# jamesmshihua/DiffusionPolicyOptimization

Measured on AMD Instinct MI355X. Metric: env-steps/sec + PPO-updates/sec, hopper-v2 64 envs 20 DDPM steps, 1/2/4/8 GPU, higher is better.
Workload: dtype bf16; 1 GPU; hopper-medium-v2 DPPO fine-tune iteration: 64 envs/GPU x 500 chunks (Ta=4), K=20 DDPM steps (K'=10), 5 PPO epochs x minibatch 50000, bf16 denoiser, synthetic linear env; env=synthetic, global_envs=64, chunks_per_rollout=500, parallelism=single GPU, batch_semantics=global minibatch 50000 rows = the reference's (50000 per rank)

## Files before the change

### diffusionpolicyoptimization_amd/_lib.py

```python
import ctypes
import os

import torch

_HERE = os.path.dirname(os.path.abspath(__file__))
LIB_PATH = os.environ.get("DPPO_LIB") or os.path.join(_HERE, "lib", "libdppo_hip.so")

DPPO_F32, DPPO_BF16, DPPO_F16 = 0, 1, 2
DPPO_ADAMW_KERAS, DPPO_ADAMW_TORCH = 0, 1
DPPO_STEP_DEFER_SAMPLER_TABLES = 0x100
DPPO_STEP_L2_FROM_PL2 = 0x200
DPPO_PPO_L2_DEFERRED = 1
DPPO_PPO_LEARN_ETA = 2
DPPO_STEP_FUSED_PACK = 0x400
DPPO_STEP_CLEAR_GRADS = 0x800
DPPO_PPO_PRECLEARED = 4
DPPO_NET_ACTOR, DPPO_NET_CRITIC = 1, 2
SCHED_COLS = 8
PRECISION = {"fp32": DPPO_F32, "f32": DPPO_F32, "bf16": DPPO_BF16, "fp16": DPPO_F16, "f16": DPPO_F16}
ACTIVATION = {"ReLU": 0, "Mish": 1}


class DppoDims(ctypes.Structure):
    _fields_ = [("obs_dim", ctypes.c_int32), ("action_dim", ctypes.c_int32), ("horizon_steps", ctypes.c_int32),
# ... 38 lines not shown
    "dppo_rollout_enqueue_tagged": (_I, [_DIMS, _I, _P, _P, _P, _P, _P, _I, _U64, _U64, _I, _I, _F, _F, _F, _P, _P,
                                         _P, ctypes.c_uint32, _P, _P]),
    "dppo_sampler_stream_bytes": (_I, [_DIMS, _I, ctypes.POINTER(ctypes.c_int64), ctypes.POINTER(ctypes.c_int)]),
    "dppo_sampler_layout": (_I, [_DIMS, _I, _I, ctypes.POINTER(ctypes.c_int)]),
    "dppo_sampler_max_in_flight": (_I, [_DIMS, _I, _I, ctypes.POINTER(ctypes.c_int)]),
    "dppo_sampler_plan": (_I, [_DIMS, _I, _I, ctypes.POINTER(ctypes.c_int)]),
    "dppo_sampler_release_stream": (_I, [_P]),
    "dppo_kernel_timing": (_I, [_I]),
    "dppo_kernel_timing_name": (ctypes.c_char_p, [_I]),
    "dppo_kernel_timing_read": (_I, [_I, _P, _P]),
    "dppo_logprob": (_I, [_DIMS, _I, _P, _P, _P, _P, _I, _F, _I, _P, _P, _P]),
    "dppo_critic_forward": (_I, [_DIMS, _I, _P, _P, _I, _P, _P]),
    "dppo_reward_scale_workspace_doubles": (_SZ, [_I, _I]),
    "dppo_reward_scale": (_I, [_P, _P, _P, _P, _P, _I, _I, _D, _D, _D, _P]),
    "dppo_reward_scale_moments": (_I, [_P, _P, _P, _P, _P, _I, _I, _D, _P]),
    "dppo_reward_scale_apply": (_I, [_P, _P, _I, _I, _D, _D, _P]),
    "dppo_reward_scale_per_env": (_I, [_P, _P, _P, _P, _I, _P, _P, _I, _I, _D, _D, _D, _P, _P]),
    "dppo_reward_scale_per_env_moments": (_I, [_P, _P, _P, _P, _P, _I, _I, _D, _P]),
    "dppo_reward_scale_per_env_apply": (_I, [_P, _P, _I, _I, _I, _D, _D, _P, _P]),
    "dppo_gae": (_I, [_P, _P, _P, _P, _I, _I, _D, _D, _D, _P, _P, _P]),
    "dppo_ppo_workspace_bytes": (_SZ, [_DIMS, _I, _I]),
    "dppo_ppo_plan": (_I, [_DIMS, _I, _I, _I, ctypes.POINTER(ctypes.c_int)]),
    "dppo_ppo_plan_act": (_I, [_DIMS, _I, _I, _I, _I, ctypes.POINTER(ctypes.c_int)]),
    "dppo_ppo_adv_stats": (_I, [_P, _I64, _I, _U64, _I, _I64, _I, _P, _P, _P]),
    "dppo_ppo_adv_stats_all": (_I, [_P, _I64, _I, _U64, _I, _I, _I64, _I, _P, _P]),
    "dppo_ppo_minibatch": (_I, [_DIMS, _I, ctypes.POINTER(DppoPpoHparams), _P, _P, _P, _P, _P, _P, _P, _P, _P,
                               _I64, _U64, _I, _I64, _I, _P, _P, _P, _P, _P, _P]),
    "dppo_pretrain_minibatch": (_I, [_DIMS, _I, _P, _P, _P, _P, _P, _P, _P, _P, _I, _I64, _F, _P, _P, _P, _P]),
    "dppo_ppo_minibatch_part": (_I, [_DIMS, _I, ctypes.POINTER(DppoPpoHparams), _P, _P, _P, _P, _P, _P, _P, _P,
                                    _P, _I64, _U64, _I, _I64, _I, _P, _P, _P, _P, _P, _I, _P]),
    "dppo_feistel_permute": (_I, [_I64, _I64, _I64, _U64, _I, _P, _P]),
    "dppo_adamw": (_I, [_P, _P, _P, _P, _I64, _I64, _F, _F, _F, _F, _F, _I, _P]),
    "dppo_copy_from_host": (_I, [_I, _P, _P, _P, _P]),
    "dppo_eta_step": (_I, [_P, _P, _I64, _F, _F, _F, _F, _F, _I, _F, _F, _P, _P, _I, _P, _P]),
    "dppo_pack_all": (_I, [_DIMS, _I, _P, _P, _P, _P, _P]),
    "dppo_optimizer_step": (_I, [_DIMS, _I, _P, _P, _P, _P, _I64, _I64, _F, _F, _F, _F, _F, _I, _P, _P, _P, _P, _P,
                                 _P, _I, _U64, _P]),
    "dppo_optimizer_step_ex": (_I, [_DIMS, _I, _P, _P, _P, _P, _I64, _I64, _F, _F, _F, _F, _F, _I, _P, _P, _P, _P,
                                    _P, _P, _I, _U64, _P, _P, _I, _P]),
    "dppo_grad_clip_workspace_bytes": (_SZ, [_DIMS, _I]),
    "dppo_grad_clip_scales": (_I, [_DIMS, _I, _P, _F, _P, _P, _P, _P]),
    "dppo_optimizer_step_clip": (_I, [_DIMS, _I, _P, _P, _P, _P, _I64, _I64, _F, _F, _F, _F, _F, _I, _P, _P, _P, _P,
                                      _P, _P, _I, _U64, _P, _P, _I, _P, _P, _I]),
    "dppo_ipc_region_bytes": (_SZ, [_I64]),
    "dppo_ipc_alloc": (_I, [_SZ, ctypes.POINTER(ctypes.c_void_p), _P]),
    "dppo_ipc_open": (_I, [_P, ctypes.POINTER(ctypes.c_void_p)]),
# ... 62 lines not shown
```

### diffusionpolicyoptimization_amd/csrc/dppo_update.h

```cpp
#pragma once
#include "dppo_ppo.h"

enum { EXTRA_NONE = 0, EXTRA_ONES = 1, EXTRA_ONEHOT = 2 };
struct DWItem {
    const void* XT; int Kx;
    const void* DT; int N;
    float* G;
    int extra;
    float* Gx;
    int nb;
};
enum class DWTile { ACTOR, CRITIC };
int launch_dw(DWTile tile, int precision, const DWItem* items, int n_items, const PpoWorkspace& ws, float out_scale,
              const int* rows_dev, int min_chunk_rows, hipStream_t s);
struct DWPlan { int tiles, nchunks, mchunk; };
DWPlan dw_plan(DWTile tile, const DWItem* items, int n_items, size_t ldm, int min_chunk_rows);

int launch_time_bwd(const Dims& D, int precision, const PpoWorkspace& ws, const void* packed_actor,
                    const float* actor_params, float* ga, int nb, int TS, hipStream_t s, bool l2_back = true);
int time_bwd_check(const Dims& D, int nb);
int launch_critic_l2_back(const Dims& D, int precision, const PpoWorkspace& ws, const void* packed_critic, float* gc,
                          uint32_t* zcnt, hipStream_t s);

struct ZeroArgs { void* p[4]; size_t n[4]; };
int launch_zero(const ZeroArgs& z, unsigned blocks, hipStream_t s);
enum { SCRATCH_TICKET = 0, SCRATCH_CRIT_COUNT = 1 };
int stream_scratch(hipStream_t s, int kind, size_t bytes, void** out);
```

### diffusionpolicyoptimization_amd/csrc/dw.hip

```cpp
#include "dppo_update.h"

#define DW_MAXP 8
#define DW_TN 128
constexpr int DW_LINE = 128;
#define DW_CPL (DW_LINE / 16)
#define DW_FPI (64 / DW_CPL)
#define DW_BOPB (DW_TN * DW_LINE)

template <int WK, int RC = 8> struct DWGeom {
    static constexpr int W = WK / 32;
    static constexpr int AOPB = WK * DW_LINE;
    static constexpr int SLOT = AOPB + DW_BOPB + 1024;
    static constexpr int RING0 = 160 * 1024 / SLOT < 8 ? 160 * 1024 / SLOT : 8;
    static constexpr int RING = RING0 < RC ? RING0 : RC;
    static constexpr int AI = WK / DW_FPI / W;
    static constexpr int BI = DW_TN / DW_FPI / W;
    static_assert(RING * SLOT <= 160 * 1024, "dW ring exceeds the CU's LDS");
};

struct DWProb {
    const void* XT; const void* DT; float* G; float* Gx;
    int Kx, N, extra, ktiles, ntiles;
    int nb;
};
struct DWArgs {
    DWProb p[DW_MAXP];
    int tile_start[DW_MAXP + 1];
    int nprob, nchunks, mchunk;
    float out_scale;
    size_t ldm;
    const int8_t* seg;
    const int* rows_dev;
};

typedef __attribute__((address_space(3))) void lds_void_t;

template <class P>
__device__ inline u32x4 extra_frag(int extra, int q, const int8_t* seg_lds) {
    using AT = typename P::AT;
    AT e[P::EPL];
    if (extra == EXTRA_ONES) {
#pragma unroll
        for (int i = 0; i < P::EPL; ++i) e[i] = P::cvt(1.f);
    } else {
        const uint64_t w = P::EPL == 8 ? *reinterpret_cast<const uint64_t*>(seg_lds)
                                       : (uint64_t)*reinterpret_cast<const uint32_t*>(seg_lds);
#pragma unroll
        for (int i = 0; i < P::EPL; ++i) e[i] = P::cvt((int)(int8_t)(w >> (8 * i)) == q ? 1.f : 0.f);
    }
    return __builtin_bit_cast(u32x4, e);
}

__device__ inline int dw_swz(int f, int c) { return c ^ (f & 7); }
__device__ inline u32x4 dw_lds_frag(const uint8_t* img, int f, int c) {
    return *reinterpret_cast<const u32x4*>(img + f * DW_LINE + (dw_swz(f, c) << 4));
}

template <int N>
__device__ inline void vm_wait() {
    static_assert(N >= 0 && N < 64, "vmcnt is 6 bits");
    __builtin_amdgcn_s_waitcnt((N & 15) | ((N >> 4) << 14) | (7 << 4) | (15 << 8));
}

template <class P, int WK, int RC, bool EXTRA, bool SEGLD>
__device__ __forceinline__ void dw_loop(uint8_t* smem, const DWArgs& a, const DWProb& pr, int nst, size_t m_begin,
                                        int wave, int lane, const typename P::AT* const (&srcA)[DWGeom<WK, RC>::AI],
                                        const typename P::AT* const (&srcB)[DWGeom<WK, RC>::BI],
                                        f32x4 (&acc)[4][4], f32x4 (&acce)[4]) {
    using G = DWGeom<WK, RC>;
    constexpr int BK = DW_LINE / (int)sizeof(typename P::AT);
    constexpr int OPS = G::AI + G::BI + (SEGLD ? 1 : 0);
    const int wr = wave >> 1, wc = wave & 1;
    const int fr = lane & 15, cq = lane >> 4;
    auto issue = [&](int st) {
        uint8_t* base = smem + (st % G::RING) * G::SLOT;
        const size_t off = (size_t)st * BK;
#pragma unroll
        for (int i = 0; i < G::AI; ++i)
            __builtin_amdgcn_global_load_lds((void*)(srcA[i] + off), (lds_void_t*)(base + (wave + G::W * i) * 1024), 16,
                                             0, 0);
#pragma unroll
        for (int i = 0; i < G::BI; ++i)
            __builtin_amdgcn_global_load_lds((void*)(srcB[i] + off),
                                             (lds_void_t*)(base + G::AOPB + (wave + G::W * i) * 1024), 16, 0, 0);
        if constexpr (SEGLD) {
            const int8_t* sg = a.seg + m_begin + off + 4 * (lane < BK / 4 ? lane : 0);
            __builtin_amdgcn_global_load_lds((void*)sg, (lds_void_t*)(base + G::AOPB + DW_BOPB), 4, 0, 0);
        }
    };
#pragma unroll
    for (int p = 0; p < G::RING - 1; ++p)
        if (p < nst) issue(p);
    for (int st = 0; st < nst; ++st) {
        const int ahead = nst - 1 - st;
        if (ahead >= G::RING - 2) vm_wait<(G::RING - 2) * OPS>();
        else if (ahead == 1) vm_wait<OPS>();
        else vm_wait<0>();
        __builtin_amdgcn_s_barrier();
        asm volatile("" ::: "memory");
        if (st + G::RING - 1 < nst) issue(st + G::RING - 1);
        const uint8_t* imA = smem + (st % G::RING) * G::SLOT;
        const uint8_t* imB = imA + G::AOPB;
        const int8_t* seg_lds = (const int8_t*)(imB + DW_BOPB);
#pragma unroll
        for (int ks = 0; ks < DW_LINE / 64; ++ks) {
            u32x4 A[4], B[4];
#pragma unroll
            for (int i = 0; i < 4; ++i) {
                A[i] = dw_lds_frag(imA, wr * 64 + i * 16 + fr, ks * 4 + cq);
                B[i] = dw_lds_frag(imB, wc * 64 + i * 16 + fr, ks * 4 + cq);
            }
#pragma unroll
            for (int i = 0; i < 4; ++i)
#pragma unroll
                for (int j = 0; j < 4; ++j) acc[i][j] = P::mma(A[i], B[j], acc[i][j]);
            if constexpr (EXTRA) {
                const u32x4 AE = extra_frag<P>(pr.extra, 16 * wr + fr, seg_lds + ks * P::KG + cq * P::EPL);
#pragma unroll
                for (int j = 0; j < 4; ++j) acce[j] = P::mma(AE, B[j], acce[j]);
            }
        }
    }
}

static int dw_device_cus() {
    static int n = [] {
        int dev = 0, c = 0;
        if (hipGetDevice(&dev) != hipSuccess || hipDeviceGetAttribute(&c, hipDeviceAttributeMultiprocessorCount, dev) != hipSuccess)
            c = 256;
        return c > 0 ? c : 256;
    }();
    return n;
}

template <class P, int WK, int RC>
__global__ __launch_bounds__(WK / 32 * 64) void dw_kernel(DWArgs a) {
    using AT = typename P::AT;
    using G = DWGeom<WK, RC>;
    constexpr int BK = DW_LINE / (int)sizeof(AT);
    constexpr int EPC = 16 / (int)sizeof(AT);
    __shared__ __attribute__((aligned(1024))) uint8_t smem[G::RING * G::SLOT];
    const int tid = threadIdx.x, lane = tid & 63, wave = tid >> 6;
    const int tiles_all = a.tile_start[a.nprob];
    const int total = tiles_all * a.nchunks;
    const int per = (total + 7) >> 3;
    const int lg = (int)(blockIdx.x & 7) * per + (int)(blockIdx.x >> 3);
    if (lg >= total) return;
    const int chunk = lg / tiles_all;
    const int tile = lg % tiles_all;
    int pi = 0;
    while (pi + 1 < a.nprob && tile >= a.tile_start[pi + 1]) ++pi;
    const DWProb& pr = a.p[pi];
    const int lt = tile - a.tile_start[pi];
    const int kt = lt / pr.ntiles, nt = lt % pr.ntiles;
    const int k_base = kt * WK, n_base = nt * DW_TN;
    const int wr = wave >> 1, wc = wave & 1;
    size_t lim = a.ldm, mchunk = (size_t)a.mchunk;
    if (a.rows_dev) {
        const size_t d64 = (size_t)(__builtin_amdgcn_readfirstlane(*a.rows_dev) + 63) / 64 * 64;
        lim = d64 < lim ? d64 : lim;
        mchunk = (lim + (size_t)a.nchunks * 64 - 1) / ((size_t)a.nchunks * 64) * 64;
    }
    const size_t m_begin = (size_t)chunk * mchunk;
    const size_t m_end = m_begin + mchunk < lim ? m_begin + mchunk : lim;
    if (m_begin >= m_end) return;
    const int nst = (int)((m_end - m_begin) / BK);
    const AT* XT = (const AT*)pr.XT;
    const AT* DT = (const AT*)pr.DT;
    const bool wg_extra = pr.extra != EXTRA_NONE && kt == 0;
    const int xrows = pr.extra == EXTRA_ONEHOT ? pr.nb : 1;
    const bool do_extra = wg_extra && 16 * wr < xrows;
    const bool seg_ld = wg_extra && wr == 0 && pr.extra == EXTRA_ONEHOT;

    const AT* srcA[G::AI];
    const AT* srcB[G::BI];
#pragma unroll
    for (int i = 0; i < G::AI; ++i) {
        const int f = (wave + G::W * i) * DW_FPI + lane / DW_CPL;
        const int c = dw_swz(f, lane % DW_CPL);
        int fa = k_base + f; fa = fa < pr.Kx ? fa : pr.Kx - 1;
        srcA[i] = XT + (size_t)fa * a.ldm + m_begin + c * EPC;
    }
#pragma unroll
    for (int i = 0; i < G::BI; ++i) {
        const int f = (wave + G::W * i) * DW_FPI + lane / DW_CPL;
        const int c = dw_swz(f, lane % DW_CPL);
        int fb = n_base + f; fb = fb < pr.N ? fb : pr.N - 1;
        srcB[i] = DT + (size_t)fb * a.ldm + m_begin + c * EPC;
    }
    f32x4 acc[4][4], acce[4];
#pragma unroll
    for (int i = 0; i < 4; ++i) {
        zero_acc(acce[i]);
#pragma unroll
        for (int j = 0; j < 4; ++j) zero_acc(acc[i][j]);
    }
    if (seg_ld) dw_loop<P, WK, RC, true, true>(smem, a, pr, nst, m_begin, wave, lane, srcA, srcB, acc, acce);
    else if (do_extra) dw_loop<P, WK, RC, true, false>(smem, a, pr, nst, m_begin, wave, lane, srcA, srcB, acc, acce);
    else dw_loop<P, WK, RC, false, false>(smem, a, pr, nst, m_begin, wave, lane, srcA, srcB, acc, acce);
#pragma unroll
    for (int i = 0; i < 4; ++i)
#pragma unroll
        for (int j = 0; j < 4; ++j) {
            const int n = n_base + wc * 64 + j * 16 + ccol(lane);
#pragma unroll
            for (int r = 0; r < 4; ++r) {
                const int k = k_base + wr * 64 + i * 16 + crow(lane, r);
                if (k < pr.Kx && n < pr.N) atomicAdd(pr.G + (size_t)k * pr.N + n, acc[i][j][r] * a.out_scale);
            }
        }
    if (do_extra) {
#pragma unroll
        for (int j = 0; j < 4; ++j) {
            const int n = n_base + wc * 64 + j * 16 + ccol(lane);
            if (n >= pr.N) continue;
#pragma unroll
            for (int r = 0; r < 4; ++r) {
                const int q = 16 * wr + crow(lane, r);
                if (pr.extra == EXTRA_ONES) {
                    if (q == 0) atomicAdd(pr.Gx + n, acce[j][r] * a.out_scale);
                } else if (q < pr.nb) {
                    atomicAdd(pr.Gx + (size_t)q * pr.N + n, acce[j][r] * a.out_scale);
                }
            }
        }
    }
}
template <class P>
static int launch_dw_p(const DWArgs& a, DWTile tile, hipStream_t s) {
    const int tiles = a.tile_start[a.nprob];
    const int64_t blocks = 8 * (((int64_t)tiles * a.nchunks + 7) / 8);
    if (tile == DWTile::ACTOR)
        hipLaunchKernelGGL((dw_kernel<P, 256, 8>), dim3((unsigned)blocks), dim3(DWGeom<256>::W * 64), 0, s, a);
    else
        hipLaunchKernelGGL((dw_kernel<P, 128, 3>), dim3((unsigned)blocks), dim3(DWGeom<128, 3>::W * 64), 0, s, a);
    DPPO_HIP(hipGetLastError());
    return DPPO_OK;
}

static int dw_item_tiles(DWTile tile, const DWItem& it) {
    return dppo_cdiv(it.Kx, tile == DWTile::ACTOR ? 256 : 128) * dppo_cdiv(it.N, DW_TN);
}

DWPlan dw_plan(DWTile tile, const DWItem* items, int n_items, size_t ldm, int min_chunk_rows) {
    DWPlan p = {};
    for (int i = 0; i < n_items; ++i) p.tiles += dw_item_tiles(tile, items[i]);
    const int span = (int)ldm;
    int nch = dw_device_cus() / p.tiles;
    if (nch > span / min_chunk_rows) nch = span / min_chunk_rows;
    if (nch < 1) nch = 1;
    p.mchunk = dppo_cdiv(span, nch * 64) * 64;
    p.nchunks = dppo_cdiv(span, p.mchunk);
    return p;
}

int launch_dw(DWTile tile, int precision, const DWItem* items, int n_items, const PpoWorkspace& ws, float out_scale,
              const int* rows_dev, int min_chunk_rows, hipStream_t s) {
    DPPO_CHECK(n_items >= 1 && n_items <= DW_MAXP, "dW: %d problems in one launch", n_items);
    const int tk = tile == DWTile::ACTOR ? 256 : 128;
    for (int i = 0; i < n_items; ++i)
        DPPO_CHECK(items[i].extra != EXTRA_ONEHOT || (items[i].nb >= 1 && items[i].nb <= tk / 4),
                   "dW: %d one-hot buckets on a %d-row tile", items[i].nb, tk);
    DWArgs w = {};
    for (int i = 0; i < n_items; ++i) {
        const DWItem& it = items[i];
        DWProb& p = w.p[i];
        p.XT = it.XT; p.DT = it.DT; p.G = it.G; p.Gx = it.Gx; p.Kx = it.Kx; p.N = it.N; p.extra = it.extra; p.nb = it.nb;
        p.ktiles = dppo_cdiv(it.Kx, tk); p.ntiles = dppo_cdiv(it.N, DW_TN);
        w.tile_start[i + 1] = w.tile_start[i] + dw_item_tiles(tile, it);
    }
    w.nprob = n_items;
    w.rows_dev = rows_dev;
    w.ldm = ws.ldm;
    w.seg = ws.seg;
    w.out_scale = out_scale;
    const DWPlan plan = dw_plan(tile, items, n_items, ws.ldm, min_chunk_rows);
    w.mchunk = plan.mchunk;
    w.nchunks = plan.nchunks;
    return precision == DPPO_BF16 ? launch_dw_p<PolicyBF16>(w, tile, s)
         : precision == DPPO_F16  ? launch_dw_p<PolicyF16>(w, tile, s) : launch_dw_p<PolicyF32>(w, tile, s);
}
```

### diffusionpolicyoptimization_amd/csrc/update.hip

```cpp
#include <stdlib.h>
#include <mutex>
#include <vector>
#include "dppo_update.h"

__global__ __launch_bounds__(256) void adv_stats_kernel(const float* __restrict__ adv, FeistelKey fk, int KF, int64_t start,
                                                        int rows, const int64_t* __restrict__ row_index,
                                                        double* __restrict__ stats) {
    __shared__ double sh[3][4];
    double c = 0.0, s = 0.0, s2 = 0.0;
    for (int64_t i = (int64_t)blockIdx.x * 256 + threadIdx.x; i < rows; i += (int64_t)gridDim.x * 256) {
        const uint64_t idx = minibatch_row(row_index, (uint64_t)(start + i), fk);
        if (idx >= fk.n) continue;
        const double v = adv[idx / KF];
        c += 1.0; s += v; s2 += v * v;
    }
    c = wave_sumd(c); s = wave_sumd(s); s2 = wave_sumd(s2);
    const int w = threadIdx.x >> 6;
    if ((threadIdx.x & 63) == 0) { sh[0][w] = c; sh[1][w] = s; sh[2][w] = s2; }
    __syncthreads();
    if (threadIdx.x == 0) {
        atomicAdd(stats + 0, sh[0][0] + sh[0][1] + sh[0][2] + sh[0][3]);
        atomicAdd(stats + 1, sh[1][0] + sh[1][1] + sh[1][2] + sh[1][3]);
        atomicAdd(stats + 2, sh[2][0] + sh[2][1] + sh[2][2] + sh[2][3]);
    }
// ... 273 lines not shown
extern "C" int dppo_ppo_plan(const dppo_dims* d, int precision, int rows, int mode, int* out) {
    return dppo_ppo_plan_act(d, precision, DPPO_ACT_RELU, rows, mode, out);
}

extern "C" int dppo_ppo_plan_act(const dppo_dims* d, int precision, int activation, int rows, int mode, int* out) {
    Dims D;
    int rc = dppo_check_dims(d, &D);
    if (rc) return rc;
    DPPO_CHECK(dppo_prec_ok(precision), "bad precision %d", precision);
    DPPO_CHECK(dppo_act_ok(activation), "dppo_ppo_plan_act: bad activation %d", activation);
    DPPO_CHECK(out && rows > 0, "dppo_ppo_plan: bad arguments");
    DPPO_CHECK(mode == DPPO_PLAN_TRAIN || mode == DPPO_PLAN_PRETRAIN || mode == DPPO_PLAN_LOGPROB,
               "dppo_ppo_plan: mode must be 0 (train), 1 (pretrain) or 2 (logprob)");
    const PpoWorkspace ws = make_ppo_workspace(D, precision, rows, nullptr);
    const ActorTilePlan t = actor_tile_plan(precision, D.H, D.XD, mode == DPPO_PLAN_LOGPROB ? (int64_t)rows : (int64_t)ws.ldm,
                                            activation);
    out[0] = 16 * t.mt;
    out[1] = t.waves;
    out[2] = out[3] = out[4] = out[5] = 0;
    if (mode == DPPO_PLAN_LOGPROB) return DPPO_OK;
    DWItem it[4];
    actor_dw_items(D, ws, nullptr, mode == DPPO_PLAN_PRETRAIN, false, it);
    const DWPlan pa = dw_plan(DWTile::ACTOR, it, 4, ws.ldm, mode == DPPO_PLAN_PRETRAIN ? PRETRAIN_MIN_CHUNK_ROWS : PPO_MIN_CHUNK_ROWS);
    out[2] = pa.nchunks;
    out[3] = pa.mchunk;
    if (mode == DPPO_PLAN_PRETRAIN) return DPPO_OK;
    critic_dw_items(D, ws, nullptr, it);
    const DWPlan pc = dw_plan(DWTile::CRITIC, it, 4, ws.ldm, PPO_MIN_CHUNK_ROWS);
    out[4] = pc.nchunks;
    out[5] = pc.mchunk;
    return DPPO_OK;
}

struct MinibatchArgs {
    const dppo_dims* d;
    int precision;
    const dppo_ppo_hparams* hp;
    const void* packed_ft; const void* packed_critic;
    const float *actor_params, *sched, *obs, *chains, *lp_old_mean, *advantages, *returns;
    int64_t total;
    uint64_t perm_seed;
    int epoch;
    int64_t start;
    int rows;
    const int64_t* row_index;
    const double* adv_stats;
    void* workspace;
    float* grads;
    double* metrics;
    void* stream;
};

static int ppo_minibatch_impl(const MinibatchArgs& m, MbPart part) {
    Dims D;
// ... 244 lines not shown
```

### diffusionpolicyoptimization_amd/ops.py

```python
import ctypes
import functools
import os
import math
import time
from dataclasses import dataclass

import numpy as np
import torch

from . import _lib
from ._lib import ptr, stream_handle


@dataclass(frozen=True)
class ModelDims:
    obs_dim: int = 11
    action_dim: int = 3
    horizon_steps: int = 4
    cond_steps: int = 1
    time_dim: int = 16
    actor_hidden: int = 512
    critic_hidden: int = 256
    denoising_steps: int = 20
    ft_denoising_steps: int = 10
# ... 667 lines not shown
def feistel_permute(first, count, n, seed, epoch, device):
    out = torch.empty(count, dtype=torch.int64, device=device)
    _lib.call("dppo_feistel_permute", int(first), int(count), int(n), ctypes.c_uint64(seed), int(epoch), ptr(out),
              stream_handle(device))
    return out


def ppo_workspace(d: ModelDims, precision, rows, device):
    nbytes = int(_lib.query("dppo_ppo_workspace_bytes", ctypes.byref(d.c()), _prec(precision), int(rows)))
    return torch.empty(nbytes, dtype=torch.uint8, device=device)


_PLAN_MODES = {"train": 0, "pretrain": 1, "logprob": 2}


def ppo_plan(d: ModelDims, precision, rows, mode="train"):
    out = (ctypes.c_int * 6)()
    _lib.call("dppo_ppo_plan_act", ctypes.byref(d.c()), _prec(precision), _lib.ACTIVATION[d.activation], int(rows),
              _PLAN_MODES[mode], out)
    return dict(actor_tile_rows=out[0], actor_waves=out[1], dw_chunks_actor=out[2], dw_chunk_rows_actor=out[3],
                dw_chunks_critic=out[4], dw_chunk_rows_critic=out[5])


def ppo_adv_stats(advantages, total, kf, perm_seed, epoch, start, rows, out, row_index=None):
    _lib.call("dppo_ppo_adv_stats", ptr(advantages), int(total), int(kf), ctypes.c_uint64(perm_seed), int(epoch),
              int(start), int(rows), ptr(row_index), ptr(out), stream_handle(advantages.device))
    return out


def ppo_adv_stats_all(advantages, total, kf, perm_seed, epoch0, n_epochs, rows_full, n_batch, out):
    _check(out, (n_epochs * n_batch, 3), torch.float64, "out")
    _lib.call("dppo_ppo_adv_stats_all", ptr(advantages), int(total), int(kf), ctypes.c_uint64(perm_seed), int(epoch0),
              int(n_epochs), int(rows_full), int(n_batch), ptr(out), stream_handle(advantages.device))
    return out


def ppo_hparams(gamma_denoising=0.99, clip_ploss_coef=0.01, clip_ploss_coef_base=0.01, clip_ploss_coef_rate=3.0,
                min_logprob_std=0.1, vf_coef=0.5, norm_adv=True, reward_horizon=4, loss_scale=1.0, global_rows=1,
                l2_deferred=False, learn_eta=False, clip_vloss_coef=None, old_values=None):
    flags = (_lib.DPPO_PPO_L2_DEFERRED if l2_deferred else 0) | (_lib.DPPO_PPO_LEARN_ETA if learn_eta else 0)
    clip = clip_vloss_coef is not None
    if clip and (old_values is None or old_values.dtype != torch.float32 or not old_values.is_cuda):
        raise ValueError("clip_vloss_coef needs the rollout's old values (fp32 device tensor)")
    if clip and not float(clip_vloss_coef) > 0:
        raise ValueError("clip_vloss_coef must be > 0")
    return _lib.DppoPpoHparams(float(gamma_denoising), float(clip_ploss_coef), float(clip_ploss_coef_base),
# ... 225 lines not shown
```

### include/dppo.h

```cpp
#ifndef DPPO_H
#define DPPO_H

#include <stddef.h>
#include <stdint.h>

#ifdef __cplusplus
extern "C" {
#endif

#define DPPO_ABI_VERSION 15

#if defined(__GNUC__)
#define DPPO_API __attribute__((visibility("default")))
#else
#define DPPO_API
#endif

enum { DPPO_OK = 0, DPPO_EINVAL = 1, DPPO_EHIP = 2, DPPO_EUNSUPPORTED = 3 };
enum { DPPO_F32 = 0, DPPO_BF16 = 1, DPPO_F16 = 2 };
enum { DPPO_ADAMW_KERAS = 0, DPPO_ADAMW_TORCH = 1 };
enum { DPPO_STEP_DEFER_SAMPLER_TABLES = 0x100 };
enum { DPPO_STEP_L2_FROM_PL2 = 0x200 };
enum { DPPO_STEP_FUSED_PACK = 0x400, DPPO_STEP_CLEAR_GRADS = 0x800 };

// ... 103 lines not shown
typedef struct dppo_ppo_hparams {
    float gamma_denoising, clip_ploss_coef, clip_ploss_coef_base, clip_ploss_coef_rate;
    float min_logprob_std, vf_coef;
    int32_t norm_adv, reward_horizon;
    float loss_scale;
    int32_t global_rows;
    int32_t flags;
    float clip_vloss_coef;
    const float* old_values;
} dppo_ppo_hparams;

enum { DPPO_PPO_L2_DEFERRED = 1 };
enum { DPPO_PPO_LEARN_ETA = 2 };
enum { DPPO_PPO_PRECLEARED = 4 };

DPPO_API int dppo_eta_step(float* eta_state, const double* metrics, int64_t step, float lr, float weight_decay,
                           float beta1, float beta2, float eps, int mode, float eta_min, float eta_max,
                           const float* ddim_base, float* sched, int ddim_steps, float* eta_out, void* stream);

DPPO_API size_t dppo_ppo_workspace_bytes(const dppo_dims* d, int precision, int batch_rows);
enum { DPPO_PLAN_TRAIN = 0, DPPO_PLAN_PRETRAIN = 1, DPPO_PLAN_LOGPROB = 2 };
DPPO_API int dppo_ppo_plan(const dppo_dims* d, int precision, int rows, int mode, int* out);
DPPO_API int dppo_ppo_plan_act(const dppo_dims* d, int precision, int activation, int rows, int mode, int* out);
DPPO_API int dppo_ppo_adv_stats(const float* advantages, int64_t total, int K_ft, uint64_t perm_seed, int epoch,
                       int64_t start, int rows, const int64_t* row_index, double* adv_stats, void* stream);
DPPO_API int dppo_ppo_adv_stats_all(const float* advantages, int64_t total, int K_ft, uint64_t perm_seed, int epoch0,
                           int n_epochs, int64_t rows_full, int n_batch, double* adv_stats, void* stream);
DPPO_API int dppo_ppo_minibatch(const dppo_dims* d, int precision, const dppo_ppo_hparams* hp,
                       const void* packed_ft, const void* packed_critic, const float* actor_params,
                       const float* sched, const float* obs, const float* chains, const float* lp_old_mean,
                       const float* advantages, const float* returns, int64_t total, uint64_t perm_seed,
                       int epoch, int64_t start, int rows, const int64_t* row_index, const double* adv_stats,
                       void* workspace, float* grads, double* metrics, void* stream);

DPPO_API int dppo_pretrain_minibatch(const dppo_dims* d, int precision, const void* packed_actor, const float* actor_params,
                            const float* sched, const float* qsched, const float* x_start, const float* cond,
                            const int32_t* t, const float* noise, int rows, int64_t global_rows, float loss_scale,
                            void* workspace, float* grads, double* metrics, void* stream);

DPPO_API int dppo_ppo_clear_ranges(const dppo_dims* d, int precision, int batch_rows, void* workspace, double* metrics,
                                   int part, void** ptrs, size_t* bytes, int* count);
DPPO_API int dppo_ppo_minibatch_part(const dppo_dims* d, int precision, const dppo_ppo_hparams* hp,
                            const void* packed_ft, const void* packed_critic, const float* actor_params,
                            const float* sched, const float* obs, const float* chains, const float* lp_old_mean,
                            const float* advantages, const float* returns, int64_t total, uint64_t perm_seed,
                            int epoch, int64_t start, int rows, const int64_t* row_index, const double* adv_stats,
// ... 52 lines not shown
```

Measured before the change: 4.145 million env-steps/s.

## Balance grouped dW kernel with per-problem chunking and narrow-tile variants

The grouped weight-gradient kernel now plans the row-chunk count per problem, using a cost model that keeps splitting the most expensive problem until the CU budget is filled, instead of applying one global chunk count. It also adds narrow A/B tile geometries for problems with small Kx or N, so tiny layers stage fewer LDS lines and run fewer MFMAs. Both aim to cut load imbalance and wasted work in the PPO backward dW launches. It adds more kernel template instantiations and per-workgroup problem lookup, plus new planning and grouped-launch entry points exposed to Python.

Measured after the change: 4.156 million env-steps/s, median of 3. No clear change (+0.3%).

```diff
diff --git a/diffusionpolicyoptimization_amd/_lib.py b/diffusionpolicyoptimization_amd/_lib.py
--- a/diffusionpolicyoptimization_amd/_lib.py
+++ b/diffusionpolicyoptimization_amd/_lib.py
@@ -84,6 +84,8 @@
     "dppo_ppo_workspace_bytes": (_SZ, [_DIMS, _I, _I]),
     "dppo_ppo_plan": (_I, [_DIMS, _I, _I, _I, ctypes.POINTER(ctypes.c_int)]),
     "dppo_ppo_plan_act": (_I, [_DIMS, _I, _I, _I, _I, ctypes.POINTER(ctypes.c_int)]),
+    "dppo_dw_plan": (_I, [_DIMS, _I, _I, _I, _I, _I, ctypes.POINTER(ctypes.c_int), ctypes.POINTER(ctypes.c_int)]),
+    "dppo_dw_grouped": (_I, [_I, _I, _I, _P, _I64, _P, _P, _I, _P, _F, _P]),
     "dppo_ppo_adv_stats": (_I, [_P, _I64, _I, _U64, _I, _I64, _I, _P, _P, _P]),
     "dppo_ppo_adv_stats_all": (_I, [_P, _I64, _I, _U64, _I, _I, _I64, _I, _P, _P]),
     "dppo_ppo_minibatch": (_I, [_DIMS, _I, ctypes.POINTER(DppoPpoHparams), _P, _P, _P, _P, _P, _P, _P, _P, _P,
diff --git a/diffusionpolicyoptimization_amd/csrc/dppo_update.h b/diffusionpolicyoptimization_amd/csrc/dppo_update.h
--- a/diffusionpolicyoptimization_amd/csrc/dppo_update.h
+++ b/diffusionpolicyoptimization_amd/csrc/dppo_update.h
@@ -1,20 +1,14 @@
 #pragma once
 #include "dppo_ppo.h"
+#include "dw_plan.h"
 
-enum { EXTRA_NONE = 0, EXTRA_ONES = 1, EXTRA_ONEHOT = 2 };
-struct DWItem {
-    const void* XT; int Kx;
-    const void* DT; int N;
-    float* G;
-    int extra;
-    float* Gx;
-    int nb;
-};
-enum class DWTile { ACTOR, CRITIC };
-int launch_dw(DWTile tile, int precision, const DWItem* items, int n_items, const PpoWorkspace& ws, float out_scale,
-              const int* rows_dev, int min_chunk_rows, hipStream_t s);
-struct DWPlan { int tiles, nchunks, mchunk; };
-DWPlan dw_plan(DWTile tile, const DWItem* items, int n_items, size_t ldm, int min_chunk_rows);
+int launch_dw(DWTile tile, int precision, const DWItem* items, int n_items, size_t ldm, const int8_t* seg, float out_scale,
+              const int* rows_dev, int min_chunk_rows, const int* nchunks, hipStream_t s);
+inline int launch_dw(DWTile tile, int precision, const DWItem* items, int n_items, const PpoWorkspace& ws, float out_scale,
+                     const int* rows_dev, int min_chunk_rows, hipStream_t s) {
+    return launch_dw(tile, precision, items, n_items, ws.ldm, ws.seg, out_scale, rows_dev, min_chunk_rows, nullptr, s);
+}
+DWPlan dw_plan(DWTile tile, const DWItem* items, int n_items, size_t ldm, int min_chunk_rows, int cus = 0);
 
 int launch_time_bwd(const Dims& D, int precision, const PpoWorkspace& ws, const void* packed_actor,
                     const float* actor_params, float* ga, int nb, int TS, hipStream_t s, bool l2_back = true);
diff --git a/diffusionpolicyoptimization_amd/csrc/dw.hip b/diffusionpolicyoptimization_amd/csrc/dw.hip
--- a/diffusionpolicyoptimization_amd/csrc/dw.hip
+++ b/diffusionpolicyoptimization_amd/csrc/dw.hip
@@ -1,32 +1,33 @@
 #include "dppo_update.h"
 
-#define DW_MAXP 8
-#define DW_TN 128
-constexpr int DW_LINE = 128;
 #define DW_CPL (DW_LINE / 16)
 #define DW_FPI (64 / DW_CPL)
-#define DW_BOPB (DW_TN * DW_LINE)
-
-template <int WK, int RC = 8> struct DWGeom {
+
+template <int WK, int RC = 8, int AL = WK, int BL = DW_TN> struct DWGeom {
     static constexpr int W = WK / 32;
-    static constexpr int AOPB = WK * DW_LINE;
-    static constexpr int SLOT = AOPB + DW_BOPB + 1024;
-    static constexpr int RING0 = 160 * 1024 / SLOT < 8 ? 160 * 1024 / SLOT : 8;
-    static constexpr int RING = RING0 < RC ? RING0 : RC;
-    static constexpr int AI = WK / DW_FPI / W;
-    static constexpr int BI = DW_TN / DW_FPI / W;
-    static_assert(RING * SLOT <= 160 * 1024, "dW ring exceeds the CU's LDS");
+    static constexpr int AOPB = AL * DW_LINE;
+    static constexpr int BOPB = BL * DW_LINE;
+    static constexpr int SLOT = dw_slot_bytes(AL, BL);
+    static constexpr int RING = dw_ring(WK, RC, AL, BL);
+    static constexpr int BYTES = dw_full_ring(WK, RC) * dw_slot_bytes(WK, DW_TN);
+    static constexpr int AIN = AL / DW_FPI, BIN = BL / DW_FPI;
+    static constexpr int AI = AIN / W;
+    static constexpr int BI = BIN >= W ? BIN / W : 1;
+    static constexpr int NJ = BL >= 64 ? 4 : 1;
+    static_assert(AIN % W == 0 && (BIN % W == 0 || W % BIN == 0), "dW stage images against the waves");
+    static_assert(RING >= 3 && RING * SLOT <= BYTES && BYTES <= 160 * 1024, "dW ring exceeds the CU's LDS");
 };
 
 struct DWProb {
     const void* XT; const void* DT; float* G; float* Gx;
     int Kx, N, extra, ktiles, ntiles;
     int nb;
+    int nchunks, mchunk;
+    int wg_start;
 };
 struct DWArgs {
     DWProb p[DW_MAXP];
-    int tile_start[DW_MAXP + 1];
-    int nprob, nchunks, mchunk;
+    int nprob, wg_total;
     float out_scale;
     size_t ldm;
     const int8_t* seg;
@@ -62,12 +63,11 @@
     __builtin_amdgcn_s_waitcnt((N & 15) | ((N >> 4) << 14) | (7 << 4) | (15 << 8));
 }
 
-template <class P, int WK, int RC, bool EXTRA, bool SEGLD>
+template <class P, class G, bool EXTRA, bool SEGLD>
 __device__ __forceinline__ void dw_loop(uint8_t* smem, const DWArgs& a, const DWProb& pr, int nst, size_t m_begin,
-                                        int wave, int lane, const typename P::AT* const (&srcA)[DWGeom<WK, RC>::AI],
-                                        const typename P::AT* const (&srcB)[DWGeom<WK, RC>::BI],
-                                        f32x4 (&acc)[4][4], f32x4 (&acce)[4]) {
-    using G = DWGeom<WK, RC>;
+                                        int wave, int lane, const typename P::AT* const (&srcA)[G::AI],
+                                        const typename P::AT* const (&srcB)[G::BI],
+                                        f32x4 (&acc)[4][G::NJ], f32x4 (&acce)[G::NJ]) {
     constexpr int BK = DW_LINE / (int)sizeof(typename P::AT);
     constexpr int OPS = G::AI + G::BI + (SEGLD ? 1 : 0);
     const int wr = wave >> 1, wc = wave & 1;
@@ -82,10 +82,10 @@
 #pragma unroll
         for (int i = 0; i < G::BI; ++i)
             __builtin_amdgcn_global_load_lds((void*)(srcB[i] + off),
-                                             (lds_void_t*)(base + G::AOPB + (wave + G::W * i) * 1024), 16, 0, 0);
+                                             (lds_void_t*)(base + G::AOPB + (wave + G::W * i) % G::BIN * 1024), 16, 0, 0);
         if constexpr (SEGLD) {
             const int8_t* sg = a.seg + m_begin + off + 4 * (lane < BK / 4 ? lane : 0);
-            __builtin_amdgcn_global_load_lds((void*)sg, (lds_void_t*)(base + G::AOPB + DW_BOPB), 4, 0, 0);
+            __builtin_amdgcn_global_load_lds((void*)sg, (lds_void_t*)(base + G::AOPB + G::BOPB), 4, 0, 0);
         }
     };
 #pragma unroll
@@ -101,23 +101,22 @@
         if (st + G::RING - 1 < nst) issue(st + G::RING - 1);
         const uint8_t* imA = smem + (st % G::RING) * G::SLOT;
         const uint8_t* imB = imA + G::AOPB;
-        const int8_t* seg_lds = (const int8_t*)(imB + DW_BOPB);
+        const int8_t* seg_lds = (const int8_t*)(imB + G::BOPB);
 #pragma unroll
         for (int ks = 0; ks < DW_LINE / 64; ++ks) {
-            u32x4 A[4], B[4];
-#pragma unroll
-            for (int i = 0; i < 4; ++i) {
-                A[i] = dw_lds_frag(imA, wr * 64 + i * 16 + fr, ks * 4 + cq);
-                B[i] = dw_lds_frag(imB, wc * 64 + i * 16 + fr, ks * 4 + cq);
-            }
+            u32x4 A[4], B[G::NJ];
+#pragma unroll
+            for (int i = 0; i < 4; ++i) A[i] = dw_lds_frag(imA, (wr * 64 + i * 16 + fr) % (G::AOPB / DW_LINE), ks * 4 + cq);
+#pragma unroll
+            for (int j = 0; j < G::NJ; ++j) B[j] = dw_lds_frag(imB, (wc * 64 + j * 16 + fr) % (G::BOPB / DW_LINE), ks * 4 + cq);
 #pragma unroll
             for (int i = 0; i < 4; ++i)
 #pragma unroll
-                for (int j = 0; j < 4; ++j) acc[i][j] = P::mma(A[i], B[j], acc[i][j]);
+                for (int j = 0; j < G::NJ; ++j) acc[i][j] = P::mma(A[i], B[j], acc[i][j]);
             if constexpr (EXTRA) {
                 const u32x4 AE = extra_frag<P>(pr.extra, 16 * wr + fr, seg_lds + ks * P::KG + cq * P::EPL);
 #pragma unroll
-                for (int j = 0; j < 4; ++j) acce[j] = P::mma(AE, B[j], acce[j]);
+                for (int j = 0; j < G::NJ; ++j) acce[j] = P::mma(AE, B[j], acce[j]);
             }
         }
     }
@@ -133,38 +132,14 @@
     return n;
 }
 
-template <class P, int WK, int RC>
-__global__ __launch_bounds__(WK / 32 * 64) void dw_kernel(DWArgs a) {
+template <class P, class G>
+__device__ __forceinline__ void dw_tile(uint8_t* smem, const DWArgs& a, const DWProb& pr, int kt, int nt, size_t m_begin,
+                                        int nst, int WK) {
     using AT = typename P::AT;
-    using G = DWGeom<WK, RC>;
-    constexpr int BK = DW_LINE / (int)sizeof(AT);
     constexpr int EPC = 16 / (int)sizeof(AT);
-    __shared__ __attribute__((aligned(1024))) uint8_t smem[G::RING * G::SLOT];
     const int tid = threadIdx.x, lane = tid & 63, wave = tid >> 6;
-    const int tiles_all = a.tile_start[a.nprob];
-    const int total = tiles_all * a.nchunks;
-    const int per = (total + 7) >> 3;
-    const int lg = (int)(blockIdx.x & 7) * per + (int)(blockIdx.x >> 3);
-    if (lg >= total) return;
-    const int chunk = lg / tiles_all;
-    const int tile = lg % tiles_all;
-    int pi = 0;
-    while (pi + 1 < a.nprob && tile >= a.tile_start[pi + 1]) ++pi;
-    const DWProb& pr = a.p[pi];
-    const int lt = tile - a.tile_start[pi];
-    const int kt = lt / pr.ntiles, nt = lt % pr.ntiles;
     const int k_base = kt * WK, n_base = nt * DW_TN;
     const int wr = wave >> 1, wc = wave & 1;
-    size_t lim = a.ldm, mchunk = (size_t)a.mchunk;
-    if (a.rows_dev) {
-        const size_t d64 = (size_t)(__builtin_amdgcn_readfirstlane(*a.rows_dev) + 63) / 64 * 64;
-        lim = d64 < lim ? d64 : lim;
-        mchunk = (lim + (size_t)a.nchunks * 64 - 1) / ((size_t)a.nchunks * 64) * 64;
-    }
-    const size_t m_begin = (size_t)chunk * mchunk;
-    const size_t m_end = m_begin + mchunk < lim ? m_begin + mchunk : lim;
-    if (m_begin >= m_end) return;
-    const int nst = (int)((m_end - m_begin) / BK);
     const AT* XT = (const AT*)pr.XT;
     const AT* DT = (const AT*)pr.DT;
     const bool wg_extra = pr.extra != EXTRA_NONE && kt == 0;
@@ -183,25 +158,25 @@
     }
 #pragma unroll
     for (int i = 0; i < G::BI; ++i) {
-        const int f = (wave + G::W * i) * DW_FPI + lane / DW_CPL;
+        const int f = (wave + G::W * i) % G::BIN * DW_FPI + lane / DW_CPL;
         const int c = dw_swz(f, lane % DW_CPL);
         int fb = n_base + f; fb = fb < pr.N ? fb : pr.N - 1;
         srcB[i] = DT + (size_t)fb * a.ldm + m_begin + c * EPC;
     }
-    f32x4 acc[4][4], acce[4];
-#pragma unroll
-    for (int i = 0; i < 4; ++i) {
-        zero_acc(acce[i]);
-#pragma unroll
-        for (int j = 0; j < 4; ++j) zero_acc(acc[i][j]);
-    }
-    if (seg_ld) dw_loop<P, WK, RC, true, true>(smem, a, pr, nst, m_begin, wave, lane, srcA, srcB, acc, acce);
-    else if (do_extra) dw_loop<P, WK, RC, true, false>(smem, a, pr, nst, m_begin, wave, lane, srcA, srcB, acc, acce);
-    else dw_loop<P, WK, RC, false, false>(smem, a, pr, nst, m_begin, wave, lane, srcA, srcB, acc, acce);
+    f32x4 acc[4][G::NJ], acce[G::NJ];
+#pragma unroll
+    for (int j = 0; j < G::NJ; ++j) {
+        zero_acc(acce[j]);
+#pragma unroll
+        for (int i = 0; i < 4; ++i) zero_acc(acc[i][j]);
+    }
+    if (seg_ld) dw_loop<P, G, true, true>(smem, a, pr, nst, m_begin, wave, lane, srcA, srcB, acc, acce);
+    else if (do_extra) dw_loop<P, G, true, false>(smem, a, pr, nst, m_begin, wave, lane, srcA, srcB, acc, acce);
+    else dw_loop<P, G, false, false>(smem, a, pr, nst, m_begin, wave, lane, srcA, srcB, acc, acce);
 #pragma unroll
     for (int i = 0; i < 4; ++i)
 #pragma unroll
-        for (int j = 0; j < 4; ++j) {
+        for (int j = 0; j < G::NJ; ++j) {
             const int n = n_base + wc * 64 + j * 16 + ccol(lane);
 #pragma unroll
             for (int r = 0; r < 4; ++r) {
@@ -211,7 +186,7 @@
         }
     if (do_extra) {
 #pragma unroll
-        for (int j = 0; j < 4; ++j) {
+        for (int j = 0; j < G::NJ; ++j) {
             const int n = n_base + wc * 64 + j * 16 + ccol(lane);
             if (n >= pr.N) continue;
 #pragma unroll
@@ -226,10 +201,42 @@
         }
     }
 }
+
+template <class P, int WK, int RC>
+__global__ __launch_bounds__(WK / 32 * 64) void dw_kernel(DWArgs a) {
+    constexpr int BK = DW_LINE / (int)sizeof(typename P::AT);
+    constexpr int NA = dw_a_lines(WK, 1);
+    __shared__ __attribute__((aligned(1024))) uint8_t smem[DWGeom<WK, RC>::BYTES];
+    const int total = a.wg_total;
+    const int per = (total + 7) >> 3;
+    const int lg = (int)(blockIdx.x & 7) * per + (int)(blockIdx.x >> 3);
+    if (lg >= total) return;
+    int pi = 0;
+    while (pi + 1 < a.nprob && lg >= a.p[pi + 1].wg_start) ++pi;
+    const DWProb& pr = a.p[pi];
+    const int tiles = pr.ktiles * pr.ntiles;
+    const int chunk = (lg - pr.wg_start) / tiles;
+    const int lt = (lg - pr.wg_start) % tiles;
+    const int kt = lt / pr.ntiles, nt = lt % pr.ntiles;
+    size_t lim = a.ldm, mchunk = (size_t)pr.mchunk;
+    if (a.rows_dev) {
+        const size_t d64 = (size_t)(__builtin_amdgcn_readfirstlane(*a.rows_dev) + 63) / 64 * 64;
+        lim = d64 < lim ? d64 : lim;
+        mchunk = (lim + (size_t)pr.nchunks * 64 - 1) / ((size_t)pr.nchunks * 64) * 64;
+    }
+    const size_t m_begin = (size_t)chunk * mchunk;
+    const size_t m_end = m_begin + mchunk < lim ? m_begin + mchunk : lim;
+    if (m_begin >= m_end) return;
+    const int nst = (int)((m_end - m_begin) / BK);
+    const bool na = dw_a_lines(WK, pr.Kx) != WK, nb = dw_b_lines(pr.N) != DW_TN;
+    if (na && nb) dw_tile<P, DWGeom<WK, RC, NA, DW_NARROW_B>>(smem, a, pr, kt, nt, m_begin, nst, WK);
+    else if (na) dw_tile<P, DWGeom<WK, RC, NA, DW_TN>>(smem, a, pr, kt, nt, m_begin, nst, WK);
+    else if (nb) dw_tile<P, DWGeom<WK, RC, WK, DW_NARROW_B>>(smem, a, pr, kt, nt, m_begin, nst, WK);
+    else dw_tile<P, DWGeom<WK, RC>>(smem, a, pr, kt, nt, m_begin, nst, WK);
+}
 template <class P>
 static int launch_dw_p(const DWArgs& a, DWTile tile, hipStream_t s) {
-    const int tiles = a.tile_start[a.nprob];
-    const int64_t blocks = 8 * (((int64_t)tiles * a.nchunks + 7) / 8);
+    const int64_t blocks = 8 * (((int64_t)a.wg_total + 7) / 8);
     if (tile == DWTile::ACTOR)
         hipLaunchKernelGGL((dw_kernel<P, 256, 8>), dim3((unsigned)blocks), dim3(DWGeom<256>::W * 64), 0, s, a);
     else
@@ -238,45 +245,41 @@
     return DPPO_OK;
 }
 
-static int dw_item_tiles(DWTile tile, const DWItem& it) {
-    return dppo_cdiv(it.Kx, tile == DWTile::ACTOR ? 256 : 128) * dppo_cdiv(it.N, DW_TN);
-}
-
-DWPlan dw_plan(DWTile tile, const DWItem* items, int n_items, size_t ldm, int min_chunk_rows) {
-    DWPlan p = {};
-    for (int i = 0; i < n_items; ++i) p.tiles += dw_item_tiles(tile, items[i]);
-    const int span = (int)ldm;
-    int nch = dw_device_cus() / p.tiles;
-    if (nch > span / min_chunk_rows) nch = span / min_chunk_rows;
-    if (nch < 1) nch = 1;
-    p.mchunk = dppo_cdiv(span, nch * 64) * 64;
-    p.nchunks = dppo_cdiv(span, p.mchunk);
-    return p;
-}
-
-int launch_dw(DWTile tile, int precision, const DWItem* items, int n_items, const PpoWorkspace& ws, float out_scale,
-              const int* rows_dev, int min_chunk_rows, hipStream_t s) {
+DWPlan dw_plan(DWTile tile, const DWItem* items, int n_items, size_t ldm, int min_chunk_rows, int cus) {
+    return dw_plan_cus(tile, items, n_items, ldm, min_chunk_rows, cus > 0 ? cus : dw_device_cus());
+}
+
+int launch_dw(DWTile tile, int precision, const DWItem* items, int n_items, size_t ldm, const int8_t* seg, float out_scale,
+              const int* rows_dev, int min_chunk_rows, const int* nchunks, hipStream_t s) {
     DPPO_CHECK(n_items >= 1 && n_items <= DW_MAXP, "dW: %d problems in one launch", n_items);
-    const int tk = tile == DWTile::ACTOR ? 256 : 128;
-    for (int i = 0; i < n_items; ++i)
+    DPPO_CHECK(ldm >= 64 && ldm % 64 == 0 && ldm < ((size_t)1 << 31), "dW: %zu rows (a multiple of 64)", ldm);
+    const int tk = dw_tile_k(tile);
+    for (int i = 0; i < n_items; ++i) {
+        DPPO_CHECK(items[i].Kx >= 1 && items[i].N >= 1, "dW: a %d x %d problem", items[i].Kx, items[i].N);
         DPPO_CHECK(items[i].extra != EXTRA_ONEHOT || (items[i].nb >= 1 && items[i].nb <= tk / 4),
                    "dW: %d one-hot buckets on a %d-row tile", items[i].nb, tk);
+    }
+    const DWPlan plan = dw_plan(tile, items, n_items, ldm, min_chunk_rows);
     DWArgs w = {};
     for (int i = 0; i < n_items; ++i) {
         const DWItem& it = items[i];
         DWProb& p = w.p[i];
         p.XT = it.XT; p.DT = it.DT; p.G = it.G; p.Gx = it.Gx; p.Kx = it.Kx; p.N = it.N; p.extra = it.extra; p.nb = it.nb;
-        p.ktiles = dppo_cdiv(it.Kx, tk); p.ntiles = dppo_cdiv(it.N, DW_TN);
-        w.tile_start[i + 1] = w.tile_start[i] + dw_item_tiles(tile, it);
+        p.ktiles = dw_cdiv(it.Kx, tk); p.ntiles = dw_cdiv(it.N, DW_TN);
+        p.nchunks = plan.nchunks[i]; p.mchunk = plan.mchunk[i];
+        if (nchunks) {
+            DPPO_CHECK(nchunks[i] >= 1 && (size_t)nchunks[i] * 64 <= ldm, "dW: %d chunks of %zu rows", nchunks[i], ldm);
+            p.mchunk = dw_cdiv((int)ldm, nchunks[i] * 64) * 64;
+            p.nchunks = dw_cdiv((int)ldm, p.mchunk);
+        }
+        p.wg_start = w.wg_total;
+        w.wg_total += p.ktiles * p.ntiles * p.nchunks;
     }
     w.nprob = n_items;
     w.rows_dev = rows_dev;
-    w.ldm = ws.ldm;
-    w.seg = ws.seg;
+    w.ldm = ldm;
+    w.seg = seg;
     w.out_scale = out_scale;
-    const DWPlan plan = dw_plan(tile, items, n_items, ws.ldm, min_chunk_rows);
-    w.mchunk = plan.mchunk;
-    w.nchunks = plan.nchunks;
     return precision == DPPO_BF16 ? launch_dw_p<PolicyBF16>(w, tile, s)
          : precision == DPPO_F16  ? launch_dw_p<PolicyF16>(w, tile, s) : launch_dw_p<PolicyF32>(w, tile, s);
 }
diff --git a/diffusionpolicyoptimization_amd/csrc/dw_plan.h b/diffusionpolicyoptimization_amd/csrc/dw_plan.h
--- /dev/null
+++ b/diffusionpolicyoptimization_amd/csrc/dw_plan.h
@@ -0,0 +1,85 @@
+#pragma once
+#include <cstddef>
+
+enum { EXTRA_NONE = 0, EXTRA_ONES = 1, EXTRA_ONEHOT = 2 };
+struct DWItem {
+    const void* XT; int Kx;
+    const void* DT; int N;
+    float* G;
+    int extra;
+    float* Gx;
+    int nb;
+};
+enum class DWTile { ACTOR, CRITIC };
+
+constexpr int DW_MAXP = 8;
+constexpr int DW_TN = 128;
+constexpr int DW_LINE = 128;
+constexpr int DW_NARROW_A = 64;
+constexpr int DW_NARROW_B = 16;
+
+constexpr int dw_tile_k(DWTile t) { return t == DWTile::ACTOR ? 256 : 128; }
+constexpr int dw_ring_cap(DWTile t) { return t == DWTile::ACTOR ? 8 : 3; }
+constexpr int dw_a_lines(int tk, int Kx) { return Kx <= DW_NARROW_A && DW_NARROW_A < tk ? DW_NARROW_A : tk; }
+constexpr int dw_b_lines(int N) { return N <= DW_NARROW_B ? DW_NARROW_B : DW_TN; }
+constexpr int dw_slot_bytes(int al, int bl) { return (al + bl) * DW_LINE + 1024; }
+constexpr int dw_full_ring(int tk, int rc) {
+    const int r = 160 * 1024 / dw_slot_bytes(tk, DW_TN) < 8 ? 160 * 1024 / dw_slot_bytes(tk, DW_TN) : 8;
+    return r < rc ? r : rc;
+}
+constexpr int dw_ring(int tk, int rc, int al, int bl) {
+    const int bytes = dw_full_ring(tk, rc) * dw_slot_bytes(tk, DW_TN);
+    return al == tk && bl == DW_TN ? dw_full_ring(tk, rc) : bytes / dw_slot_bytes(al, bl) < 8 ? bytes / dw_slot_bytes(al, bl) : 8;
+}
+
+inline int dw_cdiv(int a, int b) { return (a + b - 1) / b; }
+inline int dw_item_tiles(DWTile tile, const DWItem& it) {
+    return dw_cdiv(it.Kx, dw_tile_k(tile)) * dw_cdiv(it.N, DW_TN);
+}
+
+constexpr int DW_COST_NARROW_A = 700, DW_COST_NARROW_B = 450, DW_COST_NARROW_AB = 300;
+inline int dw_stage_cost(DWTile tile, const DWItem& it) {
+    const int tk = dw_tile_k(tile);
+    const bool na = dw_a_lines(tk, it.Kx) != tk, nb = dw_b_lines(it.N) != DW_TN;
+    if (tile != DWTile::ACTOR) return 1000;
+    return na && nb ? DW_COST_NARROW_AB : na ? DW_COST_NARROW_A : nb ? DW_COST_NARROW_B : 1000;
+}
+
+struct DWPlan {
+    int tiles, wgs, lead;
+    int ptiles[DW_MAXP], nchunks[DW_MAXP], mchunk[DW_MAXP], cost[DW_MAXP];
+};
+inline DWPlan dw_plan_cus(DWTile tile, const DWItem* items, int n_items, size_t ldm, int min_chunk_rows, int cus) {
+    DWPlan p = {};
+    const int span = (int)ldm, st = dw_cdiv(span, 64);
+    int cap = span / (min_chunk_rows > 64 ? min_chunk_rows : 64);
+    if (cap < 1) cap = 1;
+    int nch[DW_MAXP];
+    long best = -1;
+    for (int i = 0; i < n_items; ++i) {
+        p.ptiles[i] = dw_item_tiles(tile, items[i]);
+        p.cost[i] = dw_stage_cost(tile, items[i]);
+        p.tiles += p.ptiles[i];
+        nch[i] = 1;
+        if ((long)p.ptiles[i] * p.cost[i] > best) { best = (long)p.ptiles[i] * p.cost[i]; p.lead = i; }
+    }
+    p.wgs = p.tiles;
+    for (;;) {
+        int w = 0;
+        for (int i = 1; i < n_items; ++i)
+            if ((long)dw_cdiv(st, nch[i]) * p.cost[i] > (long)dw_cdiv(st, nch[w]) * p.cost[w]) w = i;
+        const int s = dw_cdiv(st, nch[w]);
+        if (s <= 1) break;
+        const int next = dw_cdiv(st, s - 1);
+        if (next > cap || p.wgs + (next - nch[w]) * p.ptiles[w] > cus) break;
+        p.wgs += (next - nch[w]) * p.ptiles[w];
+        nch[w] = next;
+    }
+    for (int i = 0; i < n_items; ++i) {
+        p.mchunk[i] = dw_cdiv(span, nch[i] * 64) * 64;
+        p.nchunks[i] = dw_cdiv(span, p.mchunk[i]);
+    }
+    p.wgs = 0;
+    for (int i = 0; i < n_items; ++i) p.wgs += p.ptiles[i] * p.nchunks[i];
+    return p;
+}
diff --git a/diffusionpolicyoptimization_amd/csrc/update.hip b/diffusionpolicyoptimization_amd/csrc/update.hip
--- a/diffusionpolicyoptimization_amd/csrc/update.hip
+++ b/diffusionpolicyoptimization_amd/csrc/update.hip
@@ -319,14 +319,56 @@
     DWItem it[4];
     actor_dw_items(D, ws, nullptr, mode == DPPO_PLAN_PRETRAIN, false, it);
     const DWPlan pa = dw_plan(DWTile::ACTOR, it, 4, ws.ldm, mode == DPPO_PLAN_PRETRAIN ? PRETRAIN_MIN_CHUNK_ROWS : PPO_MIN_CHUNK_ROWS);
-    out[2] = pa.nchunks;
-    out[3] = pa.mchunk;
+    out[2] = pa.nchunks[pa.lead];
+    out[3] = pa.mchunk[pa.lead];
+
     if (mode == DPPO_PLAN_PRETRAIN) return DPPO_OK;
     critic_dw_items(D, ws, nullptr, it);
     const DWPlan pc = dw_plan(DWTile::CRITIC, it, 4, ws.ldm, PPO_MIN_CHUNK_ROWS);
-    out[4] = pc.nchunks;
-    out[5] = pc.mchunk;
-    return DPPO_OK;
+    out[4] = pc.nchunks[pc.lead];
+    out[5] = pc.mchunk[pc.lead];
+    return DPPO_OK;
+}
+
+extern "C" int dppo_dw_plan(const dppo_dims* d, int rows, int mode, int net, int cus, int min_chunk_rows, int* n_items,
+                            int* out) {
+    Dims D;
+    int rc = dppo_check_dims(d, &D);
+    if (rc) return rc;
+    DPPO_CHECK(n_items && out && rows > 0 && cus >= 0 && min_chunk_rows >= 0, "dppo_dw_plan: bad arguments");
+    DPPO_CHECK(mode == DPPO_PLAN_TRAIN || mode == DPPO_PLAN_PRETRAIN, "dppo_dw_plan: mode must be 0 (train) or 1 (pretrain)");
+    DPPO_CHECK((net == 1 || net == 2) && !(net == 2 && mode == DPPO_PLAN_PRETRAIN),
+               "dppo_dw_plan: net must be 1 (actor) or 2 (critic, train only)");
+    const PpoWorkspace ws = make_ppo_workspace(D, DPPO_BF16, rows, nullptr);
+    DWItem it[4];
+    if (net == 1) actor_dw_items(D, ws, nullptr, mode == DPPO_PLAN_PRETRAIN, false, it);
+    else critic_dw_items(D, ws, nullptr, it);
+    if (!min_chunk_rows) min_chunk_rows = mode == DPPO_PLAN_PRETRAIN ? PRETRAIN_MIN_CHUNK_ROWS : PPO_MIN_CHUNK_ROWS;
+    const DWPlan p = dw_plan(net == 1 ? DWTile::ACTOR : DWTile::CRITIC, it, 4, ws.ldm, min_chunk_rows, cus);
+    *n_items = 4;
+    for (int i = 0; i < 4; ++i) {
+        out[4 * i] = p.ptiles[i]; out[4 * i + 1] = p.nchunks[i]; out[4 * i + 2] = p.mchunk[i]; out[4 * i + 3] = p.cost[i];
+    }
+    return DPPO_OK;
+}
+
+extern "C" int dppo_dw_grouped(int precision, int tile_rows, int n_items, const dppo_dw_item* items, int64_t ldm,
+                               const int8_t* seg, const int* rows_dev, int min_chunk_rows, const int* nchunks,
+                               float out_scale, void* stream) {
+    DPPO_CHECK(dppo_prec_ok(precision), "bad precision %d", precision);
+    DPPO_CHECK(tile_rows == 256 || tile_rows == 128, "dppo_dw_grouped: tile_rows must be 256 (actor) or 128 (critic)");
+    DPPO_CHECK(items && n_items >= 1 && n_items <= DW_MAXP && ldm > 0 && min_chunk_rows >= 64,
+               "dppo_dw_grouped: bad arguments");
+    DWItem it[DW_MAXP];
+    for (int i = 0; i < n_items; ++i) {
+        DPPO_CHECK(items[i].xt && items[i].dt && items[i].g && (items[i].extra == EXTRA_NONE || items[i].gx),
+                   "dppo_dw_grouped: item %d has a null operand", i);
+        DPPO_CHECK(items[i].extra >= EXTRA_NONE && items[i].extra <= EXTRA_ONEHOT && (items[i].extra != EXTRA_ONEHOT || seg),
+                   "dppo_dw_grouped: item %d's extra rows", i);
+        it[i] = DWItem{items[i].xt, items[i].kx, items[i].dt, items[i].n, items[i].g, items[i].extra, items[i].gx, items[i].nb};
+    }
+    return launch_dw(tile_rows == 256 ? DWTile::ACTOR : DWTile::CRITIC, precision, it, n_items, (size_t)ldm, seg, out_scale,
+                     rows_dev, min_chunk_rows, nchunks, (hipStream_t)stream);
 }
 
 struct MinibatchArgs {
diff --git a/diffusionpolicyoptimization_amd/ops.py b/diffusionpolicyoptimization_amd/ops.py
--- a/diffusionpolicyoptimization_amd/ops.py
+++ b/diffusionpolicyoptimization_amd/ops.py
@@ -713,6 +713,34 @@
                 dw_chunks_critic=out[4], dw_chunk_rows_critic=out[5])
 
 
+def dw_plan(d: ModelDims, rows, net="actor", mode="train", cus=0, min_chunk_rows=0):
+    n, out = ctypes.c_int(), (ctypes.c_int * 32)()
+    _lib.call("dppo_dw_plan", ctypes.byref(d.c()), int(rows), _PLAN_MODES[mode], {"actor": 1, "critic": 2}[net], int(cus),
+              int(min_chunk_rows), ctypes.byref(n), out)
+    return [dict(tiles=out[4 * i], chunks=out[4 * i + 1], chunk_rows=out[4 * i + 2], cost=out[4 * i + 3])
+            for i in range(n.value)]
+
+
+class DwItem(ctypes.Structure):
+    _fields_ = [("xt", ctypes.c_void_p), ("kx", ctypes.c_int32), ("dt", ctypes.c_void_p), ("n", ctypes.c_int32),
+                ("g", ctypes.c_void_p), ("extra", ctypes.c_int32), ("gx", ctypes.c_void_p), ("nb", ctypes.c_int32)]
+
+
+DW_EXTRA = {None: 0, "ones": 1, "onehot": 2}
+
+
+def dw_grouped(precision, tile_rows, items, ldm, seg=None, rows_dev=None, min_chunk_rows=768, nchunks=None, out_scale=1.0):
+    arr = (DwItem * len(items))()
+    for a, (xt, dt, g, extra, gx, nb) in zip(arr, items):
+        assert xt.shape[1] == ldm and dt.shape[1] == ldm and g.shape == (xt.shape[0], dt.shape[0])
+        assert xt.is_contiguous() and dt.is_contiguous() and g.is_contiguous() and g.dtype == torch.float32
+        a.xt, a.kx, a.dt, a.n, a.g = xt.data_ptr(), xt.shape[0], dt.data_ptr(), dt.shape[0], g.data_ptr()
+        a.extra, a.gx, a.nb = DW_EXTRA[extra], (gx.data_ptr() if gx is not None else None), int(nb)
+    nch = (ctypes.c_int * len(items))(*nchunks) if nchunks is not None else None
+    _lib.call("dppo_dw_grouped", _prec(precision), int(tile_rows), len(items), arr, int(ldm), ptr(seg), ptr(rows_dev),
+              int(min_chunk_rows), nch, float(out_scale), stream_handle(items[0][0].device))
+
+
 def ppo_adv_stats(advantages, total, kf, perm_seed, epoch, start, rows, out, row_index=None):
     _lib.call("dppo_ppo_adv_stats", ptr(advantages), int(total), int(kf), ctypes.c_uint64(perm_seed), int(epoch),
               int(start), int(rows), ptr(row_index), ptr(out), stream_handle(advantages.device))
diff --git a/include/dppo.h b/include/dppo.h
--- a/include/dppo.h
+++ b/include/dppo.h
@@ -149,6 +149,19 @@
 enum { DPPO_PLAN_TRAIN = 0, DPPO_PLAN_PRETRAIN = 1, DPPO_PLAN_LOGPROB = 2 };
 DPPO_API int dppo_ppo_plan(const dppo_dims* d, int precision, int rows, int mode, int* out);
 DPPO_API int dppo_ppo_plan_act(const dppo_dims* d, int precision, int activation, int rows, int mode, int* out);
+DPPO_API int dppo_dw_plan(const dppo_dims* d, int rows, int mode, int net, int cus, int min_chunk_rows, int* n_items,
+                          int* out);
+typedef struct dppo_dw_item {
+    const void* xt; int32_t kx;
+    const void* dt; int32_t n;
+    float* g;
+    int32_t extra;
+    float* gx;
+    int32_t nb;
+} dppo_dw_item;
+DPPO_API int dppo_dw_grouped(int precision, int tile_rows, int n_items, const dppo_dw_item* items, int64_t ldm,
+                             const int8_t* seg, const int* rows_dev, int min_chunk_rows, const int* nchunks,
+                             float out_scale, void* stream);
 DPPO_API int dppo_ppo_adv_stats(const float* advantages, int64_t total, int K_ft, uint64_t perm_seed, int epoch,
                        int64_t start, int rows, const int64_t* row_index, double* adv_stats, void* stream);
 DPPO_API int dppo_ppo_adv_stats_all(const float* advantages, int64_t total, int K_ft, uint64_t perm_seed, int epoch0,
```
